# ESCOMP/POP2-CESM

Hardware: AMD Instinct MI355X
Metric: simulated_years_per_day (higher is better)
Workload: dtype f64; 1 GPU; tx0.1v3; nt=2, steps_per_day=300, step_calls_per_day=319, distribution=equal-block-counts, blocks_local=1, hmix=del4, hmix_tracer=del4, vmix=kpp, partial_bottom_cells=False, ns_boundary=closed, grid_input=False, tadvect=centered, solver=pcg, preconditioner=diagonal, transport=none, kpp_surface_buoyancy=on-demand down to the boundary-layer depth

## Files before the change

include/pop_amd.h:

```cpp
#ifndef POP_AMD_H
#define POP_AMD_H

#ifdef __cplusplus
extern "C" {
#endif

#define POP_CONFIG_VERSION 7
typedef struct pop_config {
  int struct_version;
  int nx_global, ny_global, km, nt;
  int block_size_x, block_size_y;
  int ew_boundary;
  int ns_boundary;
  int hmix_momentum;
  int hmix_tracer;
  int lvariable_hmix;
  int vmix_choice;
  int tadvect;
  int solver_choice;
  int max_iterations;
  int convergence_check_freq;
  int tmix_opt;
  int time_mix_freq;
  int steps_per_day;
// ... 104 lines not shown
  int evp_wave;
  int fpcg_a_pair;
  int kpp_sparse;
  int pbc_generic_thomas;
  int pbc_generic_kpp;
  int stream_priority;
  int gm_sf_stored;
  int state3d_levels;
  int pcg_persist;
  int gm_flux_tile;
  int pcsi_two_step;
  int block_sums_relay;
  int pcsi_evp_fused;
  int aniso_side;
  int submeso_all_levels;
} pop_tuning;
void pop_tuning_init(pop_tuning *t);
int pop_get_tuning(const pop_ctx *ctx, pop_tuning *resolved);

int pop_create(const pop_config *cfg, int rank, int nranks, int flags, pop_ctx **out);
typedef struct pop_grid_input {
  const double *ULAT, *ULON, *HTN, *HTE, *HUS, *HUW, *ANGLE;
  const int *KMT;
  const double *DZBC;
} pop_grid_input;
int pop_create_with_grid(const pop_config *cfg, const pop_grid_input *grid, int rank, int nranks, int flags, pop_ctx **out);
int pop_create_tuned(const pop_config *cfg, const pop_grid_input *grid, const pop_tuning *tuning, int rank, int nranks, int flags, pop_ctx **out);
int pop_read_grid_files(const char *horiz_grid_file, const char *topography_file, int nx_global, int ny_global,
                        double *seven_records , int *kmt );
int pop_destroy(pop_ctx *ctx);
// ... 82 lines not shown
```

pop2-cesm_amd/csrc/kernels_barotropic.hpp:

```cpp
#pragma once
#include "kernels_common.hpp"

namespace pop {

#define POP_RED_THREADS 256

struct BtropArgs {
  const double *ZX, *ZY, *GXC, *GXO, *GYC, *GYO, *UBO, *VBO, *PCUR, *FW, *PGUESS;
  double *UH, *VH, *W3, *W4, *RHS, *centerWgt, *PNEW, *GXN, *GYN, *UBN, *VBN;
  const double *GXR, *GYR;
  const double *scal;
  double rcheck, rconst;
};
__global__ void k_btrop_rhs1(DevGrid g, StepParams sp, BtropArgs a) {
  Col c;
  if (!col_setup(g, c, false)) return;
  const long long q = c.q2;
  double W3, W4;
  if (sp.leapfrogts) {
    W3 = sp.c2dtp * (a.ZX[q] - sp.gamma * a.GXC[q] - (1.0 - sp.gamma) * a.GXO[q]);
    W4 = sp.c2dtp * (a.ZY[q] - sp.gamma * a.GYC[q] - (1.0 - sp.gamma) * a.GYO[q]);
  } else {
    W3 = sp.c2dtp * (a.ZX[q] - a.GXC[q]);
    W4 = sp.c2dtp * (a.ZY[q] - a.GYC[q]);
// ... 600 lines not shown

}

namespace pop {

struct FusedArgs {
  double *X, *R, *Z, *S0, *S1, *Q;
  double *AZ; const double *A0R;
  const double *Bv, *C;
  double *partA, *partB;
  SolverScalars *sc;
  const int *srcmap;
  int nchunk, nblocks;
  const double *bsA, *bsB;
  int presummed;
  const int *sendmap, *send_off, *send_slot;
  double *sendbuf;
  const int *rmap;
  const double *rbuf;
};
__device__ __forceinline__ bool send_band(const DevGrid &g, int b, int i, int j) {
  return i + 1 < g.ib + NGHOST || i + 1 > blk_ie(g, b) - NGHOST || j + 1 < g.jb + NGHOST || j + 1 > blk_je(g, b) - NGHOST;
}
__device__ __forceinline__ void pack_cell(const FusedArgs &a, long long q, double val) {
  const int e = a.sendmap[q];
  if (e < 0) return;
  for (int n = a.send_off[e]; n < a.send_off[e + 1]; ++n) a.sendbuf[a.send_slot[n]] = val;
}
__device__ __forceinline__ double z_at(const FusedArgs &a, int m) {
  if (a.rmap) { const int rs = a.rmap[m]; if (rs >= 0) return a.rbuf[rs]; }
  return a.Z[m];
}

template <class T>
__device__ __forceinline__ T sld(const T *p) { return *(const __attribute__((address_space(4))) T *)p; }
__device__ __forceinline__ double presummed_total(const double *__restrict__ bs, int nblocks) {
  double total = 0.0;
  for (int b = 0; b < nblocks; ++b) total = total + sld(bs + b);
  return total;
}
__device__ __forceinline__ double fused_total(const double *__restrict__ partial, int nchunk, int nblocks,
                                              const double *__restrict__ bs, int presummed) {
  __shared__ double shf[POP_RED_THREADS];
  __shared__ double shf_tot;
  const int t = threadIdx.x;
  double total = 0.0;
  if (presummed) return presummed_total(bs, nblocks);
  for (int b = 0; b < nblocks; ++b) {
    double v = 0.0;
    for (int c = t; c < nchunk; c += POP_RED_THREADS) v = v + partial[(long long)b * nchunk + c];
    shf[t] = v;
    __syncthreads();
    if (t < 64) { const double x = tree_tail64((shf[t] + shf[t + 128]) + (shf[t + 64] + shf[t + 192])); if (t == 0) shf_tot = x; }
    __syncthreads();
    total = total + shf_tot;
  }
  return total;
}

constexpr unsigned long long POP_SPIN_EMPTY = 0x7FF8DEADBEEF0001ULL;

// ... 314 lines not shown
    a.X[q] = x + al * s;
    const double rn = r - al * qq;
    a.R[q] = rn;
    if (a.sendmap && send_band(g, b, i, j)) pack_cell(a, q, rn * a.A0R[q]);
  } else if (live && a.rmap) {
    const int rs = a.rmap[q];
    if (rs >= 0) {
      const double sg = a.rbuf[rs] + bt * a.S0[q];
      a.S0[q] = sg;
      a.X[q] = a.X[q] + al * sg;
    }
  }
}

template <bool XUPD>
__global__ void __launch_bounds__(POP_RED_THREADS / 2)
k_fpcg_b2(DevGrid g, FusedArgs a) {
  const int stop = sld(&a.sc->stop);
  const double alpha = XUPD ? sld(&a.sc->alpha) : 0.0;
  const double eta0 = sld(&a.sc->eta0);
  const double rz = presummed_total(a.bsA, a.nblocks);
  if (red_land_out<1>(g, a.partB, a.nchunk, a.sendmap != nullptr)) return;
  __shared__ double sh[POP_RED_THREADS];
  const int b = blockIdx.y, t = threadIdx.x, nxb = g.nxb;
  const long long p0 = (long long)red_chunk(g) * POP_RED_THREADS + 2 * t;
  const bool live0 = p0 < g.n2, live1 = p0 + 1 < g.n2;
  const int pp = live0 ? (int)p0 : 0;
  const int i = pp % nxb, j = pp / nxb;
  const long long q = (long long)b * g.n2 + pp;
  const bool fast = live1 && i + 1 > g.ib && i + 2 < blk_ie(g, b) && j + 1 > g.jb && j + 1 < blk_je(g, b);
  double v0 = 0.0, v1 = 0.0;
  double zr[3][4], sr[3][4];
  double2 cc, xx, x0, xm, y0, ym;
  double x0w = 0.0, xmw = 0.0, y0w = 0.0, ymw = 0.0, mk0 = 0.0, mk1 = 0.0;
  if (fast) {
#pragma unroll
    for (int r = 0; r < 3; ++r) {
      const long long o = q + (long long)(r - 1) * nxb;
      const double2 zc = *reinterpret_cast<const double2 *>(a.Z + o), sc = *reinterpret_cast<const double2 *>(a.S0 + o);
      zr[r][0] = a.Z[o - 1]; zr[r][1] = zc.x; zr[r][2] = zc.y; zr[r][3] = a.Z[o + 2];
      sr[r][0] = a.S0[o - 1]; sr[r][1] = sc.x; sr[r][2] = sc.y; sr[r][3] = a.S0[o + 2];
    }
    cc = *reinterpret_cast<const double2 *>(a.C + q);
    x0 = *reinterpret_cast<const double2 *>(g.XW + q); xm = *reinterpret_cast<const double2 *>(g.XW + q - nxb);
    y0 = *reinterpret_cast<const double2 *>(g.YW + q); ym = *reinterpret_cast<const double2 *>(g.YW + q - nxb);
    x0w = g.XW[q - 1]; xmw = g.XW[q - 1 - nxb]; y0w = g.YW[q - 1]; ymw = g.YW[q - 1 - nxb];
    mk0 = (double)g.mMask8[q]; mk1 = (double)g.mMask8[q + 1];
    if (XUPD) xx = *reinterpret_cast<const double2 *>(a.X + q);
  }
  if (stop) return;
  const double bt = rz / eta0;
  if (blockIdx.x == 0 && blockIdx.y == 0 && t == 0) { a.sc->eta1 = rz; a.sc->beta_cg = bt; }
  if (fast) {
    if (XUPD) *reinterpret_cast<double2 *>(a.X + q) = make_double2(xx.x + alpha * sr[1][1], xx.y + alpha * sr[1][2]);
    double2 no0, nom, ea0, ne0, nem;
    const double ne0w = x0w + y0w, nemw = xmw + ymw;
    ne0.x = x0.x + y0.x; ne0.y = x0.y + y0.y; nem.x = xm.x + ym.x; nem.y = xm.y + ym.y;
    const double eaw = x0w + xmw - y0w - ymw;
    ea0.x = x0.x + xm.x - y0.x - ym.x; ea0.y = x0.y + xm.y - y0.y - ym.y;
    no0.x = y0.x + y0w - x0.x - x0w; no0.y = y0.y + y0.x - x0.y - x0.x;
    nom.x = ym.x + ymw - xm.x - xmw; nom.y = ym.y + ym.x - xm.y - xm.x;
#define SN(r, c) (zr[r][c] + sr[r][c] * bt)
    const double sA = SN(1, 1), sB = SN(1, 2);
    double aqA = cc.x * sA;
    aqA = aqA + no0.x * SN(2, 1); aqA = aqA + nom.x * SN(0, 1); aqA = aqA + ea0.x * SN(1, 2); aqA = aqA + eaw * SN(1, 0);
    aqA = aqA + ne0.x * SN(2, 2); aqA = aqA + nem.x * SN(0, 2); aqA = aqA + ne0w * SN(2, 0); aqA = aqA + nemw * SN(0, 0);
    double aqB = cc.y * sB;
    aqB = aqB + no0.y * SN(2, 2); aqB = aqB + nom.y * SN(0, 2); aqB = aqB + ea0.y * SN(1, 3); aqB = aqB + ea0.x * SN(1, 1);
    aqB = aqB + ne0.y * SN(2, 3); aqB = aqB + nem.y * SN(0, 3); aqB = aqB + ne0.x * SN(2, 1); aqB = aqB + nem.x * SN(0, 1);
#undef SN
    *reinterpret_cast<double2 *>(a.S1 + q) = make_double2(sA, sB);
    *reinterpret_cast<double2 *>(a.Q + q) = make_double2(aqA, aqB);
    v0 = (aqA * sA) * mk0; v1 = (aqB * sB) * mk1;
  } else {
    const int off[9] = {0, nxb, -nxb, 1, -1, nxb + 1, -nxb + 1, nxb - 1, -nxb - 1};
    const long long qsafe = (long long)b * g.n2 + nxb + 1;
#pragma unroll
    for (int e = 0; e < 2; ++e) {
      const bool live = (e == 0 ? live0 : live1);
      const int p2 = live ? (int)(p0 + e) : 0, ii = p2 % nxb, jj = p2 / nxb;
      const long long qq = (long long)b * g.n2 + p2;
      const bool in_e = live && interior(g, b, ii, jj);
      const long long qn = in_e ? qq : qsafe;
      const double sold = a.S0[qq], xold = XUPD ? a.X[qq] : 0.0;
      const double zown = in_e ? a.Z[qq] : z_at(a, (int)qq);
      int m[9];
#pragma unroll
      for (int n = 1; n < 9; ++n) m[n] = a.srcmap[qn + off[n]];
      const double wv[9] = {a.C[qn], g.WNo[qn], g.WNo[qn - nxb], g.WEa[qn], g.WEa[qn - 1], g.WNE[qn], g.WNE[qn - nxb], g.WNE[qn - 1], g.WNE[qn - 1 - nxb]};
      const double mk = (double)g.mMask8[qn];
      double zn[9], sn0[9];
#pragma unroll
      for (int n = 1; n < 9; ++n) { const int mm = (m[n] >= 0) ? m[n] : (int)qn; zn[n] = z_at(a, mm); sn0[n] = a.S0[mm]; }
      const double s = zown + sold * bt;
      double aq = 0.0, vv = 0.0;
      if (in_e) {
        aq = wv[0] * s;
#pragma unroll
        for (int n = 1; n < 9; ++n) {
          const double sn = (m[n] >= 0) ? zn[n] + sn0[n] * bt : 0.0 + 0.0 * bt;
          aq = aq + wv[n] * sn;
        }
        vv = (aq * s) * mk;
      }
      if (live) {
        if (XUPD) a.X[qq] = xold + alpha * sold;
        a.S1[qq] = s; a.Q[qq] = aq;
      }
      if (e == 0) v0 = vv; else v1 = vv;
    }
  }
  sh[2 * t] = v0; sh[2 * t + 1] = v1;
  __syncthreads();
  if (t < 64) {
    const double x = tree_tail64((sh[t] + sh[t + 128]) + (sh[t + 64] + sh[t + 192]));
    if (t == 0) a.partB[(long long)b * a.nchunk + red_chunk(g)] = x;
  }
}

__global__ void __launch_bounds__(POP_RED_THREADS)
k_fpcg_xr(DevGrid g, FusedArgs a) {
  if (a.sc->stop) return;
  if (red_land(g, a.sendmap != nullptr)) return;
  const int p2 = red_cell(g), b = blockIdx.y;
  const double sq = fused_total(a.partB, a.nchunk, a.nblocks, a.bsB, a.presummed);
  const double rz = a.sc->eta1;
  const double alpha = rz / sq;
  if (blockIdx.x == 0 && blockIdx.y == 0 && threadIdx.x == 0) { a.sc->eta0 = rz; a.sc->alpha = alpha; }
  if (p2 >= g.n2) return;
  const long long q = (long long)b * g.n2 + p2;
  a.X[q] = a.X[q] + alpha * a.S0[q];
}

template <bool WITH_RR>
__global__ void __launch_bounds__(POP_RED_THREADS)
k_fresidual(DevGrid g, FusedArgs a) {
  if (a.sc->stop) return;
  if (WITH_RR ? red_land_out<1>(g, a.partA, a.nchunk, a.sendmap != nullptr) : red_land(g, a.sendmap != nullptr)) return;
  const int p2 = red_cell(g), b = blockIdx.y;
  double v[1] = {0.0};
// ... 116 lines not shown
```

pop2-cesm_amd/csrc/launch_solvers.hpp:

```cpp
#pragma once

namespace {

SolverArgs solver_args(pop_ctx *c) {
  SolverArgs a{};
  a.X = c->PS[c->newt]; a.R = c->R; a.S0 = c->S0; a.S1 = c->S1; a.Q = c->Q; a.Z = c->Z; a.AZ = c->AZ;
  a.Bv = c->RHS; a.C = c->centerWgt; a.partial = c->partial; a.sc = c->sc;
  return a;
}

int evp_apply(pop_ctx *c, const double *X, double *PX, bool residual = true) {
  const int wave = tun_or(c->h.tun.evp_wave, 3);
  if (wave == 3 && c->evp.C0 && residual)
    hipLaunchKernelGGL(k_evp_apply_wave3<true>, dim3((unsigned)((c->evp.S + POP_EVP_SB - 1) / POP_EVP_SB)), dim3(64), 0, c->stream, c->evp, c->g.nxb, X, PX);
  else if (wave == 3 && c->evp.C0)
    hipLaunchKernelGGL(k_evp_apply_wave3<false>, dim3((unsigned)((c->evp.S + POP_EVP_SB - 1) / POP_EVP_SB)), dim3(64), 0, c->stream, c->evp, c->g.nxb, X, PX);
  else if (wave == 2 && c->evp.C0)
    hipLaunchKernelGGL(k_evp_apply_wave2, dim3((unsigned)((c->evp.S + POP_EVP_SB - 1) / POP_EVP_SB)), dim3(64), 0, c->stream, c->evp, c->g.nxb, X, PX);
  else if (wave != 0)
    hipLaunchKernelGGL(k_evp_apply_wave, dim3((unsigned)((c->evp.S + POP_EVP_SB - 1) / POP_EVP_SB)), dim3(64), 0, c->stream, c->evp, c->g.nxb, X, PX);
  else
    hipLaunchKernelGGL(k_evp_apply, dim3((unsigned)((c->evp.S + POP_EVP_THREADS - 1) / POP_EVP_THREADS)), dim3(POP_EVP_THREADS), 0, c->stream,
                       c->evp, c->g.nxb, X, PX);
  HIPCHK(c, hipGetLastError());
// ... 51 lines not shown
      if (read_scalars(c, &s)) return 1;
      rr = s.rr;
      if (rr < c->h.convergenceCriterion) { c->numIterations = m; break; }
    }
  }
  if (pending) { a = solver_args(c); hipLaunchKernelGGL(k_pcg_xr, G, B, 0, c->stream, c->g, a); }
  return solver_finish(c, nullptr, nullptr, 0, rr, "POP_SolversPCG");
}

static bool fpcg_pair_ok(const pop_ctx *c, const SolveView &v, const FusedArgs &a) {
  return v.g.red_act && a.presummed && !a.sendmap && (v.g.red_nact % 16) == 0 && !tun_off(c->h.tun.fpcg_b2) && !tun_off(c->h.tun.fpcg_a_pair);
}
static bool presum_by_size(long long nchunk, long long nblocks) { return nchunk * nblocks > 2048; }
static bool two_cell_shape(const DevGrid &g, bool presummed) { return presummed && (g.nxb & 1) == 0 && !g.red_tiles; }
static bool two_cell_ok(const pop_ctx *c, const DevGrid &g, bool presummed) { return two_cell_shape(g, presummed) && !tun_off(c->h.tun.fpcg_b2); }
FusedArgs fused_args(pop_ctx *c, const SolveView &v) {
  FusedArgs a{};
  a.X = v.X; a.R = v.R; a.Z = v.Z; a.S0 = v.S0; a.S1 = v.S1; a.Q = v.Q;
  a.Bv = v.RHS; a.C = v.C; a.partA = v.partial; a.partB = v.partial + (size_t)v.nchunk * v.g.nblocks;
  a.sc = c->sc; a.srcmap = v.srcmap; a.nchunk = v.nchunk; a.nblocks = v.g.nblocks;
  a.bsA = v.blocksum + 2 * v.nblocks_tot; a.bsB = v.blocksum + 3 * v.nblocks_tot;
  a.presummed = (presum_by_size(v.nchunk, v.g.nblocks) || tun_on(c->h.tun.solver_presum)) ? 1 : 0;
  return a;
}
constexpr int POP_RELAY_LMAX = 36;
static bool presum_relay(const pop_ctx *c, const SolveView &v) {
  const int terms = (v.nchunk + POP_RED_THREADS - 1) / POP_RED_THREADS;
  const int t = tun_or(c->h.tun.block_sums_relay, 1);
  return (terms > 64 || t == 2) && (terms + 3) / 4 <= POP_RELAY_LMAX && t != 0;
}
template <int NF = 1>
void presum(pop_ctx *c, const SolveView &v, const double *partial, double *bs) {
  if (presum_relay(c, v)) hipLaunchKernelGGL((k_block_sums_relay<NF, POP_RELAY_LMAX>), dim3(v.g.nblocks, NF), dim3(1024), 0, c->stream, partial, v.nchunk, (const int *)c->iota, bs);
  else hipLaunchKernelGGL(k_block_sums<NF>, dim3(v.g.nblocks), dim3(POP_RED_THREADS), 0, c->stream, partial, v.nchunk, (const int *)c->iota, bs);
}
dim3 view_grid(const SolveView &v) { return dim3(red_grid_x(v.g), v.g.nblocks); }
template <bool WITH_RR>
// ... 13 lines not shown
    else hipLaunchKernelGGL(k_fpcg_a_pair<false>, GP, B, 0, c->stream, v.g, a);
  } else if (update) hipLaunchKernelGGL(k_fpcg_a<true>, G, B, 0, c->stream, v.g, a);
  else hipLaunchKernelGGL(k_fpcg_a<false>, G, B, 0, c->stream, v.g, a);
}
void launch_fpcg_b(pop_ctx *c, const SolveView &v, const FusedArgs &a, bool xupd) {
  const dim3 G = view_grid(v);
  const bool two = two_cell_ok(c, v.g, a.presummed != 0);
  if (two && xupd) hipLaunchKernelGGL(k_fpcg_b2<true>, G, dim3(POP_RED_THREADS / 2), 0, c->stream, v.g, a);
  else if (two) hipLaunchKernelGGL(k_fpcg_b2<false>, G, dim3(POP_RED_THREADS / 2), 0, c->stream, v.g, a);
  else if (xupd) hipLaunchKernelGGL(k_fpcg_b<true>, G, dim3(POP_RED_THREADS), 0, c->stream, v.g, a);
  else hipLaunchKernelGGL(k_fpcg_b<false>, G, dim3(POP_RED_THREADS), 0, c->stream, v.g, a);
}
void fused_iterations(pop_ctx *c, SolveView &v, int n, bool pending) {
  for (int it = 0; it < n; ++it) {
    FusedArgs a = fused_args(c, v);
    launch_fpcg_a(c, v, a, pending);
    if (a.presummed) presum(c, v, a.partA, (double *)a.bsA);
    launch_fpcg_b(c, v, a, pending);
    if (a.presummed) presum(c, v, a.partB, (double *)a.bsB);
    std::swap(v.S0, v.S1);
    pending = true;
  }
}
int fused_interval(pop_ctx *c, SolveView &v, int freq) {
  const dim3 G = view_grid(v), B(POP_RED_THREADS);
  fused_iterations(c, v, freq, false);
  FusedArgs a = fused_args(c, v);
  hipLaunchKernelGGL(k_fpcg_xr, G, B, 0, c->stream, v.g, a);
  launch_fresidual<true>(c, v, a);
  hipLaunchKernelGGL(k_rr_total, dim3(1), dim3(POP_RED_THREADS), 0, c->stream, (const double *)v.partial, v.nchunk, v.g.nblocks, c->sc, c->host_rr, c->h.convergenceCriterion);
// ... 173 lines not shown
}
int persist_give_up(pop_ctx *c, const char *instead, const SolveView &v, const double *X0) {
  c->persist_gave_up += 1;
  fprintf(stderr, "libpop_amd: %s -- continuing with %s\n", c->err.c_str(), instead);
  c->err.clear();
  if (X0) HIPCHK(c, hipMemcpyAsync(v.X, X0, sizeof(double) * v.g.n2 * v.g.nblocks, hipMemcpyDeviceToDevice, c->stream));
  return 0;
}
int persist_keep_x0(pop_ctx *c, const SolveView &v, const pop_ctx::PersistPlan &pl) {
  HIPCHK(c, hipMemcpyAsync(pl.X0, v.X, sizeof(double) * v.g.n2 * v.g.nblocks, hipMemcpyDeviceToDevice, c->stream));
  return 0;
}

int solver_pcg_fused(pop_ctx *c, SolveView &v) {
  const pop_config &cf = c->h.c;
  c->persist_used = 0;
  if (!tun_off(c->h.tun.pcg_persist) && !fused_args(c, v).presummed) {
    const pop_ctx::PersistPlan *pl = c->persist_gave_up ? nullptr : persist_plan(c, v);
    if (pl) {
      static void (*const kern[4])(PersistArgs) = {k_pcg_persist<1>, k_pcg_persist<2>, k_pcg_persist<4>, k_pcg_persist<8>};
      if (persist_keep_x0(c, v, *pl)) return 1;
      const int e = persist_launch(c, v, *pl, persist_args(c, v, *pl), kern, "resident pcg", "POP_SolversPCG");
      if (e != 3) return e;
      if (persist_give_up(c, "the two-launch pcg", v, pl->X0)) return 1;
    }
  }
  const dim3 G = view_grid(v), B(POP_RED_THREADS);
  const int freq = cf.convergence_check_freq;
  if (solver_begin(c, 1.0)) return 1;
  HIPCHK(c, hipMemsetAsync(v.S0, 0, sizeof(double) * v.g.n2 * v.g.nblocks, c->stream));
  launch_fresidual<false>(c, v, fused_args(c, v));
  c->numIterations = cf.max_iterations;
// ... 587 lines not shown
```

pop2-cesm_amd/csrc/pop_amd.hip:

```cpp
#include <hip/hip_runtime.h>
#include <algorithm>
#include <chrono>
#include <unordered_map>
#include "kernels_baroclinic.hpp"
#include "kernels_barotropic.hpp"
#include "kernels_mix.hpp"
#include "kernels_thomas_reg.hpp"
#include "kernels_momentum_lds.hpp"
#include "kernels_aniso.hpp"
#include "kernels_submeso.hpp"
#include "kernels_tracer_lds.hpp"
#include "kernels_rf.hpp"
#include "kernels_pcsi.hpp"
#include "kernels_evp.hpp"
#include "kernels_lwlim.hpp"
#include "kernels_gm.hpp"
#include "kernels_pcg_persist.hpp"
#include <fcntl.h>
#include <unistd.h>
#include "rccl_transport.hpp"

using namespace pop;

#include "pop_ctx.hpp"
// ... 79 lines not shown
  return pop_create_tuned(cfg, grid, nullptr, rank, nranks, flags, out);
}

#define POP_TUNING_FIELDS(X)                                                                                                            \
  X(land_skip, "POP_LAND_SKIP") X(land_full_steps, "POP_LAND_FULL_STEPS") X(xcd_remap, "POP_XCD_REMAP") X(red_tiles, "POP_RED_TILES")   \
  X(red_band, "POP_RED_BAND") X(lds_order, "POP_LDS_ORDER") X(momentum_lds, "POP_MOMENTUM_LDS") X(tracer_lds, "POP_TRACER_LDS")         \
  X(generic_thomas, "POP_GENERIC_THOMAS") X(reg_thomas_t, "POP_REG_THOMAS_T") X(thomas_pair, "POP_THOMAS_PAIR")                         \
  X(tracer_fwd, "POP_TRACER_FWD") X(vdc_shared, "POP_VDC_SHARED") X(side_stream, "POP_SIDE_STREAM") X(del4_side, "POP_DEL4_SIDE")       \
  X(del4_tile, "POP_DEL4_TILE") X(d2t_fuse, "POP_D2T_FUSE") X(d2u_fuse, "POP_D2U_FUSE") X(vmixu_defer, "POP_VMIXU_DEFER")               \
  X(vmixu_inline, "POP_VMIXU_INLINE") X(btrop_inline, "POP_BTROP_INLINE") X(kpp_ahead, "POP_KPP_AHEAD") X(kpp_col, "POP_KPP_COL")       \
  X(kpp_lazy, "POP_KPP_LAZY") X(kpp_ushear_hint, "POP_KPP_USHEAR_HINT") X(kpp_ushear_margin, "POP_KPP_USHEAR_MARGIN")                   \
  X(kpp_side_stream, "POP_KPP_SIDE_STREAM") X(kpp_buoy_waves, "POP_KPP_BUOY_WAVES") X(kpp_interior_generic, "POP_KPP_INTERIOR_GENERIC") \
  X(kpp_src_full, "POP_KPP_SRC_FULL") X(solver_unfused, "POP_SOLVER_UNFUSED") X(solver_nograph, "POP_SOLVER_NOGRAPH")                   \
  X(solver_presum, "POP_SOLVER_PRESUM") X(solver_distributed, "POP_SOLVER_DISTRIBUTED") X(solver_overlap_off, "POP_SOLVER_OVERLAP_OFF") \
  X(fpcg_b2, "POP_FPCG_B2") X(pcsi_step2, "POP_PCSI_STEP2") X(halo_separate, "POP_HALO_SEPARATE")                                       \
  X(halo_overlap_off, "POP_HALO_OVERLAP_OFF") X(rccl_overlap, "POP_RCCL_OVERLAP") X(evp_wave, "POP_EVP_WAVE") X(fpcg_a_pair, "POP_FPCG_A_PAIR") X(stream_priority, "POP_STREAM_PRIORITY") X(kpp_sparse, "POP_KPP_SPARSE") X(pbc_generic_thomas, "POP_PBC_GENERIC_THOMAS") X(pbc_generic_kpp, "POP_PBC_GENERIC_KPP") X(state3d_levels, "POP_STATE3D_LEVELS") X(gm_sf_stored, "POP_GM_SF_STORED") X(pcg_persist, "POP_PCG_PERSIST") X(gm_flux_tile, "POP_GM_FLUX_TILE") X(pcsi_two_step, "POP_PCSI_TWO_STEP") X(block_sums_relay, "POP_BLOCK_SUMS_RELAY") X(pcsi_evp_fused, "POP_PCSI_EVP_FUSED") X(aniso_side, "POP_ANISO_SIDE") X(submeso_all_levels, "POP_SUBMESO_ALL_LEVELS")
void pop_tuning_init(pop_tuning *t) {
  if (!t) return;
  t->struct_bytes = (int)sizeof(pop_tuning);
#define X(f, e) t->f = POP_TUNING_UNSET;
  POP_TUNING_FIELDS(X)
#undef X
}
static void tuning_resolve(pop_tuning &t, const pop_tuning *user) {
  pop_tuning_init(&t);
  if (user && user->struct_bytes == (int)sizeof(pop_tuning)) t = *user;
  auto env = [](const char *name, int &v) {
    const char *e = getenv(name);
    if (!e) return;
    char *end = nullptr;
    const long x = strtol(e, &end, 10);
// ... 439 lines not shown
      for (size_t w = act[b].size(); w < longest; ++w) seq.push_back(land[b][w - act[b].size()]);
      const size_t per = longest / 8;
      for (size_t w = 0; w < longest; ++w) list[(size_t)b * longest + (w % per) * 8 + w / per] = seq[w];
    }
    if (!can_pad) longest = (size_t)nc;
    if (longest < (size_t)nc) {
      std::vector<int> cnt(h.nblocks);
      for (int b = 0; b < h.nblocks; ++b) cnt[b] = (int)act[b].size();
      if (dev_upload(c, &c->red_act, list.data(), list.size()) || dev_upload(c, &c->red_cnt, cnt.data(), cnt.size())) return 1;
      c->red_nact = (int)longest;
    }
  }
  if (dev_alloc(c, &c->partial, (size_t)c->nchunk * h.nblocks * 2 + POP_RELAY_SLACK) || dev_alloc(c, &c->blocksum, (size_t)h.nblocks_tot * 4)) return 1;
  { std::vector<int> io(h.nblocks_tot); for (int b = 0; b < h.nblocks_tot; ++b) io[b] = b; if (dev_upload(c, &c->iota, io.data(), io.size())) return 1; }
  if (dev_alloc(c, &c->sc, 1)) return 1;
  { std::vector<int> gid(h.nblocks); for (int lb = 0; lb < h.nblocks; ++lb) gid[lb] = h.local_ids[lb] - 1; if (dev_upload(c, &c->gid, gid.data(), gid.size())) return 1; }
  { std::vector<int> log(h.nblocks_tot, -1); for (int lb = 0; lb < h.nblocks; ++lb) log[h.local_ids[lb] - 1] = lb; if (dev_upload(c, &c->loc_of_gid, log.data(), log.size())) return 1; }
  c->ncopy = (int)h.halo.copy_dst.size(); c->nfill = (int)h.halo.fill_dst.size();
  if (c->ncopy && (dev_upload(c, &c->copy_dst, h.halo.copy_dst.data(), c->ncopy) || dev_upload(c, &c->copy_src, h.halo.copy_src.data(), c->ncopy))) return 1;
  if (c->nfill && dev_upload(c, &c->fill_dst, h.halo.fill_dst.data(), c->nfill)) return 1;
  for (auto &pp : h.halo.peers) {
    DevPeer d; d.rank = pp.rank; d.nsend = (int)pp.send_src.size(); d.nrecv = (int)pp.recv_dst.size();
    if (d.nsend && dev_upload(c, &d.send_src, pp.send_src.data(), d.nsend)) return 1;
    if (d.nrecv && dev_upload(c, &d.recv_dst, pp.recv_dst.data(), d.nrecv)) return 1;
    c->peers.push_back(d);
  }
  if (cfg->ns_boundary == 2) {
    size_t nmax = 1;
    for (int loc = 0; loc < 5; ++loc) {
      const TripolePlan &T = h.halo.tripole[loc];
// ... 248 lines not shown
  if (n == "d2t_fused") return c->d2t_next[0] != nullptr;
  if (n == "d2u_fused") return c->d2u_next[0] != nullptr;
  if (n == "d2t_last_formed") return c->d2t_last_formed;
  if (n == "d2u_last_formed") return c->d2u_last_formed;
  if (n == "avg_ts") return c->avg_ts;
  if (n == "nsteps_total") return c->nsteps_total;
  if (n == "nsteps_per_interval") return c->h.nsteps_per_interval;
  if (n == "solver_stream_ops") return (int)c->solver_ops;
  if (n == "solver_iterations_enqueued") return (int)c->solver_enq;
  if (n == "rank") return c->h.rank;
  if (n == "nranks") return c->h.nranks;
  if (n == "solver_chunks_per_block") return c->nchunk;
  if (n == "solver_chunks_listed") return c->red_act ? c->red_nact : -1;
  if (n == "solver_chunks_active") return c->red_active_total;
  if (n == "pcg_persist_used") return c->persist_used;
  if (n == "pcg_persist_gave_up") return c->persist_gave_up;
  if (n == "pcsi_evp_fused") return c->pcsi_evp_fused ? 1 : 0;
  if (n == "pcsi_two_step") return (c->pcsi_two_step || c->pcsi_two_step_dist) ? 1 : 0;
  if (n == "pcg_persist_workgroups") return c->persist_nwg;
  if (n == "pcg_persist_chunks_per_workgroup") return c->persist_cp;
  if (n == "solver_path") return c->host_only ? 0 : solver_path_code(c);
  if (n == "thomas_register_tracers") return c->reg_thomas_t && (c->g.km == 60 || c->g.km == 62);
  if (n == "thomas_register_velocity") return c->reg_thomas && (c->g.km == 60 || c->g.km == 62);
  if (n == "max_blocks_per_rank") return c->max_blocks_per_rank;
  if (n == "ocean_columns_local") return (int)c->h.ocean_cols_local;
  if (n == "ocean_columns_total") return (int)c->h.ocean_cols_total;
  return -1;
}
double pop_get_scalar(const pop_ctx *c, const char *name) {
  const std::string n(name);
// ... 1340 lines not shown
```

pop2-cesm_amd/csrc/pop_ctx.hpp:

```cpp
#pragma once

#define HIPCHK(ctx, call)                                                                       \
  do {                                                                                          \
    hipError_t e_ = (call);                                                                     \
    if (e_ != hipSuccess) {                                                                     \
      (ctx)->err = std::string(#call) + ": " + hipGetErrorString(e_);                           \
      return 1;                                                                                 \
    }                                                                                           \
  } while (0)

struct PhaseTimer { double ms = 0; int calls = 0; };

struct DevPeer { int rank; int *send_src = nullptr, *recv_dst = nullptr; int nsend = 0, nrecv = 0; };

struct pop_ctx {
  HostModel h;
  bool host_only = true;
  std::string err;
  hipStream_t stream = nullptr;
  bool own_stream = false;
  DevGrid g{};
  std::map<std::string, double *> d2;
  std::map<std::string, int *> di2;
  std::vector<void *> allocs;
// ... 41 lines not shown
  struct PersistPlan {
    const void *key = nullptr; bool ok = false; std::string why;
    int CP = 0, nwg = 0, nwin_max = 0, nslots = 0;
    int *own_q = nullptr, *halo_off = nullptr, *halo_q = nullptr; unsigned short *nbr = nullptr;
    PWord *W = nullptr;
    double *X0 = nullptr;
  };
  unsigned long long persist_epoch = 0;
  std::vector<PersistPlan> persist;
  std::vector<int> h_srcmap;
  double *persist_out = nullptr;
  int persist_used = 0;
  int persist_gave_up = 0;
  int red_active_total = 0;
  int persist_nwg = 0, persist_cp = 0;
  bool pcsi_two_cell = false;
  bool pcsi_two_step = false;
  bool pcsi_two_step_dist = false;
  double *pcsi_raw = nullptr;
  int *pcsi_jfold = nullptr;
  bool pcsi_evp_fused = false;
  bool reg_thomas_t = true;
  int trc_lds_rows = 4;
  int mom_lds_rows = 4;
  bool reg_thomas = true;
  SolveView gv{};
  double *gTAREA = nullptr; int *gKMT = nullptr;
  int nchunk = 0, numIterations = 0;
  double rmsResidual = 0.0;
  int *copy_dst = nullptr, *copy_src = nullptr, *fill_dst = nullptr;
// ... 111 lines not shown
```

Baseline: 10.22 SYPD.

## Add accumulator-owner fused PCG kernels that replace per-iteration presum reduction launches

```diff
diff --git a/include/pop_amd.h b/include/pop_amd.h
--- a/include/pop_amd.h
+++ b/include/pop_amd.h
@@ -142,6 +142,7 @@
   int pcsi_evp_fused;
   int aniso_side;
   int submeso_all_levels;
+  int fpcg_acc_owner;
 } pop_tuning;
 void pop_tuning_init(pop_tuning *t);
 int pop_get_tuning(const pop_ctx *ctx, pop_tuning *resolved);
diff --git a/pop2-cesm_amd/csrc/kernels_barotropic.hpp b/pop2-cesm_amd/csrc/kernels_barotropic.hpp
--- a/pop2-cesm_amd/csrc/kernels_barotropic.hpp
+++ b/pop2-cesm_amd/csrc/kernels_barotropic.hpp
@@ -638,6 +638,7 @@
   int nchunk, nblocks;
   const double *bsA, *bsB;
   int presummed;
+  double *accA, *accB;
   const int *sendmap, *send_off, *send_slot;
   double *sendbuf;
   const int *rmap;
@@ -663,12 +664,27 @@
   for (int b = 0; b < nblocks; ++b) total = total + sld(bs + b);
   return total;
 }
+__device__ __forceinline__ double acc_total(const double *__restrict__ acc, int nblocks) {
+  const int l = threadIdx.x & 63;
+  double total = 0.0;
+  for (int b = 0; b < nblocks; ++b) {
+    const double *__restrict__ v = acc + (long long)b * POP_RED_THREADS;
+    const double x = tree_tail64((v[l] + v[l + 128]) + (v[l + 64] + v[l + 192]));
+    total = total + __shfl(x, 0, 64);
+  }
+  return total;
+}
 __device__ __forceinline__ double fused_total(const double *__restrict__ partial, int nchunk, int nblocks,
-                                              const double *__restrict__ bs, int presummed) {
+                                              const double *__restrict__ bs, int presummed, const double *__restrict__ acc = nullptr) {
   __shared__ double shf[POP_RED_THREADS];
   __shared__ double shf_tot;
   const int t = threadIdx.x;
   double total = 0.0;
+  if (acc) {
+    if (t < 64) { const double x = acc_total(acc, nblocks); if (t == 0) shf_tot = x; }
+    __syncthreads();
+    return shf_tot;
+  }
   if (presummed) return presummed_total(bs, nblocks);
   for (int b = 0; b < nblocks; ++b) {
     double v = 0.0;
@@ -1013,6 +1029,120 @@
 }
 
 template <bool XUPD>
+struct FpcgBPair {
+  long long p0, q;
+  int nxb;
+  bool live0, live1, fast;
+  double zr[3][4], sr[3][4];
+  double2 cc, xx, x0, xm, y0, ym;
+  double x0w, xmw, y0w, ymw, mk0, mk1;
+  __device__ __forceinline__ void setup(const DevGrid &g, int b, int chunk, int tt) {
+    nxb = g.nxb;
+    p0 = (long long)chunk * POP_RED_THREADS + 2 * tt;
+    live0 = p0 < g.n2; live1 = p0 + 1 < g.n2;
+    const int pp = live0 ? (int)p0 : 0;
+    const int i = pp % nxb, j = pp / nxb;
+    q = (long long)b * g.n2 + pp;
+    fast = live1 && i + 1 > g.ib && i + 2 < blk_ie(g, b) && j + 1 > g.jb && j + 1 < blk_je(g, b);
+    x0w = 0.0; xmw = 0.0; y0w = 0.0; ymw = 0.0; mk0 = 0.0; mk1 = 0.0;
+  }
+  __device__ __forceinline__ void load(const DevGrid &g, const FusedArgs &a, int b, int chunk, int tt) {
+    setup(g, b, chunk, tt);
+    if (fast) load_fast(g, a);
+  }
+  __device__ __forceinline__ void finish(const DevGrid &g, const FusedArgs &a, int b, double bt, double alpha, double &v0, double &v1) {
+    if (fast) finish_fast(a, bt, alpha, v0, v1);
+    else finish_generic(g, a, b, bt, alpha, v0, v1);
+  }
+  __device__ __forceinline__ void run(const DevGrid &g, const FusedArgs &a, int b, int chunk, int tt, double bt, double alpha, double &v0, double &v1) {
+    setup(g, b, chunk, tt);
+    if (fast) { load_fast(g, a); finish_fast(a, bt, alpha, v0, v1); }
+    else finish_generic(g, a, b, bt, alpha, v0, v1);
+  }
+  __device__ __forceinline__ void load_fast(const DevGrid &g, const FusedArgs &a) {
+    {
+#pragma unroll
+      for (int r = 0; r < 3; ++r) {
+        const long long o = q + (long long)(r - 1) * nxb;
+        const double2 zc = *reinterpret_cast<const double2 *>(a.Z + o), sc = *reinterpret_cast<const double2 *>(a.S0 + o);
+        zr[r][0] = a.Z[o - 1]; zr[r][1] = zc.x; zr[r][2] = zc.y; zr[r][3] = a.Z[o + 2];
+        sr[r][0] = a.S0[o - 1]; sr[r][1] = sc.x; sr[r][2] = sc.y; sr[r][3] = a.S0[o + 2];
+      }
+      cc = *reinterpret_cast<const double2 *>(a.C + q);
+      x0 = *reinterpret_cast<const double2 *>(g.XW + q); xm = *reinterpret_cast<const double2 *>(g.XW + q - nxb);
+      y0 = *reinterpret_cast<const double2 *>(g.YW + q); ym = *reinterpret_cast<const double2 *>(g.YW + q - nxb);
+      x0w = g.XW[q - 1]; xmw = g.XW[q - 1 - nxb]; y0w = g.YW[q - 1]; ymw = g.YW[q - 1 - nxb];
+      mk0 = (double)g.mMask8[q]; mk1 = (double)g.mMask8[q + 1];
+      if (XUPD) xx = *reinterpret_cast<const double2 *>(a.X + q);
+    }
+  }
+  __device__ __forceinline__ void finish_fast(const FusedArgs &a, double bt, double alpha, double &v0, double &v1) {
+    {
+      if (XUPD) *reinterpret_cast<double2 *>(a.X + q) = make_double2(xx.x + alpha * sr[1][1], xx.y + alpha * sr[1][2]);
+      double2 no0, nom, ea0, ne0, nem;
+      const double ne0w = x0w + y0w, nemw = xmw + ymw;
+      ne0.x = x0.x + y0.x; ne0.y = x0.y + y0.y; nem.x = xm.x + ym.x; nem.y = xm.y + ym.y;
+      const double eaw = x0w + xmw - y0w - ymw;
+      ea0.x = x0.x + xm.x - y0.x - ym.x; ea0.y = x0.y + xm.y - y0.y - ym.y;
+      no0.x = y0.x + y0w - x0.x - x0w; no0.y = y0.y + y0.x - x0.y - x0.x;
+      nom.x = ym.x + ymw - xm.x - xmw; nom.y = ym.y + ym.x - xm.y - xm.x;
+#define SN(r, c) (zr[r][c] + sr[r][c] * bt)
+      const double sA = SN(1, 1), sB = SN(1, 2);
+      double aqA = cc.x * sA;
+      aqA = aqA + no0.x * SN(2, 1); aqA = aqA + nom.x * SN(0, 1); aqA = aqA + ea0.x * SN(1, 2); aqA = aqA + eaw * SN(1, 0);
+      aqA = aqA + ne0.x * SN(2, 2); aqA = aqA + nem.x * SN(0, 2); aqA = aqA + ne0w * SN(2, 0); aqA = aqA + nemw * SN(0, 0);
+      double aqB = cc.y * sB;
+      aqB = aqB + no0.y * SN(2, 2); aqB = aqB + nom.y * SN(0, 2); aqB = aqB + ea0.y * SN(1, 3); aqB = aqB + ea0.x * SN(1, 1);
+      aqB = aqB + ne0.y * SN(2, 3); aqB = aqB + nem.y * SN(0, 3); aqB = aqB + ne0.x * SN(2, 1); aqB = aqB + nem.x * SN(0, 1);
+#undef SN
+      *reinterpret_cast<double2 *>(a.S1 + q) = make_double2(sA, sB);
+      *reinterpret_cast<double2 *>(a.Q + q) = make_double2(aqA, aqB);
+      v0 = (aqA * sA) * mk0; v1 = (aqB * sB) * mk1;
+    }
+  }
+  __device__ __forceinline__ void finish_generic(const DevGrid &g, const FusedArgs &a, int b, double bt, double alpha, double &v0, double &v1) {
+    v0 = 0.0; v1 = 0.0;
+    {
+      const int off[9] = {0, nxb, -nxb, 1, -1, nxb + 1, -nxb + 1, nxb - 1, -nxb - 1};
+      const long long qsafe = (long long)b * g.n2 + nxb + 1;
+#pragma unroll
+      for (int e = 0; e < 2; ++e) {
+        const bool live = (e == 0 ? live0 : live1);
+        const int p2 = live ? (int)(p0 + e) : 0, ii = p2 % nxb, jj = p2 / nxb;
+        const long long qq = (long long)b * g.n2 + p2;
+        const bool in_e = live && interior(g, b, ii, jj);
+        const long long qn = in_e ? qq : qsafe;
+        const double sold = a.S0[qq], xold = XUPD ? a.X[qq] : 0.0;
+        const double zown = in_e ? a.Z[qq] : z_at(a, (int)qq);
+        int m[9];
+#pragma unroll
+        for (int n = 1; n < 9; ++n) m[n] = a.srcmap[qn + off[n]];
+        const double wv[9] = {a.C[qn], g.WNo[qn], g.WNo[qn - nxb], g.WEa[qn], g.WEa[qn - 1], g.WNE[qn], g.WNE[qn - nxb], g.WNE[qn - 1], g.WNE[qn - 1 - nxb]};
+        const double mk = (double)g.mMask8[qn];
+        double zn[9], sn0[9];
+#pragma unroll
+        for (int n = 1; n < 9; ++n) { const int mm = (m[n] >= 0) ? m[n] : (int)qn; zn[n] = z_at(a, mm); sn0[n] = a.S0[mm]; }
+        const double s = zown + sold * bt;
+        double aq = 0.0, vv = 0.0;
+        if (in_e) {
+          aq = wv[0] * s;
+#pragma unroll
+          for (int n = 1; n < 9; ++n) {
+            const double sn = (m[n] >= 0) ? zn[n] + sn0[n] * bt : 0.0 + 0.0 * bt;
+            aq = aq + wv[n] * sn;
+          }
+          vv = (aq * s) * mk;
+        }
+        if (live) {
+          if (XUPD) a.X[qq] = xold + alpha * sold;
+          a.S1[qq] = s; a.Q[qq] = aq;
+        }
+        if (e == 0) v0 = vv; else v1 = vv;
+      }
+    }
+  }
+};
+template <bool XUPD>
 __global__ void __launch_bounds__(POP_RED_THREADS / 2)
 k_fpcg_b2(DevGrid g, FusedArgs a) {
   const int stop = sld(&a.sc->stop);
@@ -1021,94 +1151,14 @@
   const double rz = presummed_total(a.bsA, a.nblocks);
   if (red_land_out<1>(g, a.partB, a.nchunk, a.sendmap != nullptr)) return;
   __shared__ double sh[POP_RED_THREADS];
-  const int b = blockIdx.y, t = threadIdx.x, nxb = g.nxb;
-  const long long p0 = (long long)red_chunk(g) * POP_RED_THREADS + 2 * t;
-  const bool live0 = p0 < g.n2, live1 = p0 + 1 < g.n2;
-  const int pp = live0 ? (int)p0 : 0;
-  const int i = pp % nxb, j = pp / nxb;
-  const long long q = (long long)b * g.n2 + pp;
-  const bool fast = live1 && i + 1 > g.ib && i + 2 < blk_ie(g, b) && j + 1 > g.jb && j + 1 < blk_je(g, b);
-  double v0 = 0.0, v1 = 0.0;
-  double zr[3][4], sr[3][4];
-  double2 cc, xx, x0, xm, y0, ym;
-  double x0w = 0.0, xmw = 0.0, y0w = 0.0, ymw = 0.0, mk0 = 0.0, mk1 = 0.0;
-  if (fast) {
-#pragma unroll
-    for (int r = 0; r < 3; ++r) {
-      const long long o = q + (long long)(r - 1) * nxb;
-      const double2 zc = *reinterpret_cast<const double2 *>(a.Z + o), sc = *reinterpret_cast<const double2 *>(a.S0 + o);
-      zr[r][0] = a.Z[o - 1]; zr[r][1] = zc.x; zr[r][2] = zc.y; zr[r][3] = a.Z[o + 2];
-      sr[r][0] = a.S0[o - 1]; sr[r][1] = sc.x; sr[r][2] = sc.y; sr[r][3] = a.S0[o + 2];
-    }
-    cc = *reinterpret_cast<const double2 *>(a.C + q);
-    x0 = *reinterpret_cast<const double2 *>(g.XW + q); xm = *reinterpret_cast<const double2 *>(g.XW + q - nxb);
-    y0 = *reinterpret_cast<const double2 *>(g.YW + q); ym = *reinterpret_cast<const double2 *>(g.YW + q - nxb);
-    x0w = g.XW[q - 1]; xmw = g.XW[q - 1 - nxb]; y0w = g.YW[q - 1]; ymw = g.YW[q - 1 - nxb];
-    mk0 = (double)g.mMask8[q]; mk1 = (double)g.mMask8[q + 1];
-    if (XUPD) xx = *reinterpret_cast<const double2 *>(a.X + q);
-  }
+  const int b = blockIdx.y, t = threadIdx.x;
+  FpcgBPair<XUPD> P;
+  P.load(g, a, b, red_chunk(g), t);
   if (stop) return;
   const double bt = rz / eta0;
   if (blockIdx.x == 0 && blockIdx.y == 0 && t == 0) { a.sc->eta1 = rz; a.sc->beta_cg = bt; }
-  if (fast) {
-    if (XUPD) *reinterpret_cast<double2 *>(a.X + q) = make_double2(xx.x + alpha * sr[1][1], xx.y + alpha * sr[1][2]);
-    double2 no0, nom, ea0, ne0, nem;
-    const double ne0w = x0w + y0w, nemw = xmw + ymw;
-    ne0.x = x0.x + y0.x; ne0.y = x0.y + y0.y; nem.x = xm.x + ym.x; nem.y = xm.y + ym.y;
-    const double eaw = x0w + xmw - y0w - ymw;
-    ea0.x = x0.x + xm.x - y0.x - ym.x; ea0.y = x0.y + xm.y - y0.y - ym.y;
-    no0.x = y0.x + y0w - x0.x - x0w; no0.y = y0.y + y0.x - x0.y - x0.x;
-    nom.x = ym.x + ymw - xm.x - xmw; nom.y = ym.y + ym.x - xm.y - xm.x;
-#define SN(r, c) (zr[r][c] + sr[r][c] * bt)
-    const double sA = SN(1, 1), sB = SN(1, 2);
-    double aqA = cc.x * sA;
-    aqA = aqA + no0.x * SN(2, 1); aqA = aqA + nom.x * SN(0, 1); aqA = aqA + ea0.x * SN(1, 2); aqA = aqA + eaw * SN(1, 0);
-    aqA = aqA + ne0.x * SN(2, 2); aqA = aqA + nem.x * SN(0, 2); aqA = aqA + ne0w * SN(2, 0); aqA = aqA + nemw * SN(0, 0);
-    double aqB = cc.y * sB;
-    aqB = aqB + no0.y * SN(2, 2); aqB = aqB + nom.y * SN(0, 2); aqB = aqB + ea0.y * SN(1, 3); aqB = aqB + ea0.x * SN(1, 1);
-    aqB = aqB + ne0.y * SN(2, 3); aqB = aqB + nem.y * SN(0, 3); aqB = aqB + ne0.x * SN(2, 1); aqB = aqB + nem.x * SN(0, 1);
-#undef SN
-    *reinterpret_cast<double2 *>(a.S1 + q) = make_double2(sA, sB);
-    *reinterpret_cast<double2 *>(a.Q + q) = make_double2(aqA, aqB);
-    v0 = (aqA * sA) * mk0; v1 = (aqB * sB) * mk1;
-  } else {
-    const int off[9] = {0, nxb, -nxb, 1, -1, nxb + 1, -nxb + 1, nxb - 1, -nxb - 1};
-    const long long qsafe = (long long)b * g.n2 + nxb + 1;
-#pragma unroll
-    for (int e = 0; e < 2; ++e) {
-      const bool live = (e == 0 ? live0 : live1);
-      const int p2 = live ? (int)(p0 + e) : 0, ii = p2 % nxb, jj = p2 / nxb;
-      const long long qq = (long long)b * g.n2 + p2;
-      const bool in_e = live && interior(g, b, ii, jj);
-      const long long qn = in_e ? qq : qsafe;
-      const double sold = a.S0[qq], xold = XUPD ? a.X[qq] : 0.0;
-      const double zown = in_e ? a.Z[qq] : z_at(a, (int)qq);
-      int m[9];
-#pragma unroll
-      for (int n = 1; n < 9; ++n) m[n] = a.srcmap[qn + off[n]];
-      const double wv[9] = {a.C[qn], g.WNo[qn], g.WNo[qn - nxb], g.WEa[qn], g.WEa[qn - 1], g.WNE[qn], g.WNE[qn - nxb], g.WNE[qn - 1], g.WNE[qn - 1 - nxb]};
-      const double mk = (double)g.mMask8[qn];
-      double zn[9], sn0[9];
-#pragma unroll
-      for (int n = 1; n < 9; ++n) { const int mm = (m[n] >= 0) ? m[n] : (int)qn; zn[n] = z_at(a, mm); sn0[n] = a.S0[mm]; }
-      const double s = zown + sold * bt;
-      double aq = 0.0, vv = 0.0;
-      if (in_e) {
-        aq = wv[0] * s;
-#pragma unroll
-        for (int n = 1; n < 9; ++n) {
-          const double sn = (m[n] >= 0) ? zn[n] + sn0[n] * bt : 0.0 + 0.0 * bt;
-          aq = aq + wv[n] * sn;
-        }
-        vv = (aq * s) * mk;
-      }
-      if (live) {
-        if (XUPD) a.X[qq] = xold + alpha * sold;
-        a.S1[qq] = s; a.Q[qq] = aq;
-      }
-      if (e == 0) v0 = vv; else v1 = vv;
-    }
-  }
+  double v0, v1;
+  P.finish(g, a, b, bt, alpha, v0, v1);
   sh[2 * t] = v0; sh[2 * t + 1] = v1;
   __syncthreads();
   if (t < 64) {
@@ -1117,12 +1167,134 @@
   }
 }
 
+constexpr int POP_ACC_THREADS = 1024;
+constexpr int POP_ACC_MAXTERMS = 1024;
+__device__ __forceinline__ int acc_of_workgroup(int w) { return (w & 7) * (POP_RED_THREADS / 8) + (w >> 3); }
+__device__ __forceinline__ bool own_land(const DevGrid &g, int b, int k) {
+  return g.skip && !(b == 0 && k == 0) && land_run(g, b, (long long)k * POP_RED_THREADS, POP_RED_THREADS);
+}
+__device__ __forceinline__ double wave_uniform(double x) {
+  const long long u = __double_as_longlong(x);
+  const unsigned lo = __builtin_amdgcn_readfirstlane((unsigned)u), hi = __builtin_amdgcn_readfirstlane((unsigned)(u >> 32));
+  return __longlong_as_double((long long)(((unsigned long long)hi << 32) | lo));
+}
+template <class F>
+__device__ __forceinline__ void own_chunks(const DevGrid &g, int b, int acc, int nchunk, double *part, F chunk_partial) {
+  const int l = threadIdx.x & 63, wave = __builtin_amdgcn_readfirstlane((int)(threadIdx.x >> 6)), nwaves = (int)(blockDim.x >> 6);
+  int turn = 0;
+  for (int m0 = 0; acc + POP_RED_THREADS * m0 < nchunk; m0 += 64) {
+    const int chl = acc + POP_RED_THREADS * (m0 + l);
+    const bool there = chl < nchunk, land = there && own_land(g, b, chl);
+    if (wave == 0 && land) part[m0 + l] = 0.0;
+    unsigned long long todo = __ballot(there && !land);
+    while (todo) {
+      const int bit = __ffsll(todo) - 1;
+      todo &= todo - 1;
+      const bool mine = turn % nwaves == wave;
+      ++turn;
+      if (mine) {
+        const double x = chunk_partial(acc + POP_RED_THREADS * (m0 + bit));
+        if (l == 0) part[m0 + bit] = x;
+      }
+    }
+  }
+}
+__device__ __forceinline__ void own_store_acc(const double *part, int acc, int nchunk, double *__restrict__ out) {
+  if (threadIdx.x != 0) return;
+  const int terms = (nchunk - acc + POP_RED_THREADS - 1) / POP_RED_THREADS;
+  double v = 0.0;
+  int m = 0;
+  for (; m + 16 <= terms; m += 16) {
+    double w[16];
+#pragma unroll
+    for (int u = 0; u < 16; ++u) w[u] = part[m + u];
+#pragma unroll
+    for (int u = 0; u < 16; ++u) v = v + w[u];
+  }
+  for (; m < terms; ++m) v = v + part[m];
+  *out = v;
+}
+template <bool UPDATE>
+__global__ void __launch_bounds__(POP_ACC_THREADS)
+k_fpcg_a_own(DevGrid g, FusedArgs a) {
+  __shared__ double part[POP_ACC_MAXTERMS];
+  if (sld(&a.sc->stop)) return;
+  const int b = blockIdx.y, l = threadIdx.x & 63, acc = acc_of_workgroup(blockIdx.x);
+  double alpha = 0.0;
+  if (UPDATE) {
+    const double sq = acc_total(a.accB, a.nblocks);
+    const double rz = sld(&a.sc->eta1);
+    alpha = wave_uniform(rz / sq);
+    if (blockIdx.x == 0 && blockIdx.y == 0 && threadIdx.x == 0) { a.sc->eta0 = rz; a.sc->alpha = alpha; }
+  }
+  own_chunks(g, b, acc, a.nchunk, part, [&](int ch) {
+    long long q[4]; bool live[4];
+    double r[4], qq[4] = {0.0, 0.0, 0.0, 0.0}, cw[4], mk[4], v[4];
+#pragma unroll
+    for (int u = 0; u < 4; ++u) {
+      const long long p2 = (long long)ch * POP_RED_THREADS + l + 64 * u;
+      live[u] = p2 < g.n2;
+      q[u] = (long long)b * g.n2 + (live[u] ? p2 : 0);
+    }
+#pragma unroll
+    for (int u = 0; u < 4; ++u) {
+      r[u] = a.R[q[u]];
+      if (UPDATE) qq[u] = a.Q[q[u]];
+      cw[u] = a.C[q[u]]; mk[u] = (double)g.mMask8[q[u]];
+    }
+#pragma unroll
+    for (int u = 0; u < 4; ++u) {
+      v[u] = 0.0;
+      if (live[u]) {
+        const int p2 = (int)(q[u] - (long long)b * g.n2);
+        const int i = p2 % g.nxb, j = p2 / g.nxb;
+        double rr = r[u];
+        if (UPDATE) { rr = rr - alpha * qq[u]; a.R[q[u]] = rr; }
+        const double z = (cw[u] != 0.0) ? rr / cw[u] : 0.0;
+        a.Z[q[u]] = z;
+        if (interior(g, b, i, j)) v[u] = (rr * z) * mk[u];
+      }
+    }
+    return tree_tail64((v[0] + v[2]) + (v[1] + v[3]));
+  });
+  __syncthreads();
+  own_store_acc(part, acc, a.nchunk, a.accA + (long long)b * POP_RED_THREADS + acc);
+}
+template <bool XUPD>
+__global__ void __launch_bounds__(POP_ACC_THREADS)
+k_fpcg_b_own(DevGrid g, FusedArgs a) {
+  __shared__ double part[POP_ACC_MAXTERMS];
+  if (sld(&a.sc->stop)) return;
+  const double alpha = XUPD ? sld(&a.sc->alpha) : 0.0;
+  const double eta0 = sld(&a.sc->eta0);
+  const int b = blockIdx.y, l = threadIdx.x & 63, acc = acc_of_workgroup(blockIdx.x);
+  const double rz = acc_total(a.accA, a.nblocks);
+  const double bt = wave_uniform(rz / eta0);
+  if (blockIdx.x == 0 && blockIdx.y == 0 && threadIdx.x == 0) { a.sc->eta1 = rz; a.sc->beta_cg = bt; }
+  const bool odd = (l & 1) != 0;
+  own_chunks(g, b, acc, a.nchunk, part, [&](int ch) {
+    double s02 = 0.0, s13 = 0.0;
+#pragma unroll 1
+    for (int h = 0; h < 2; ++h) {
+      FpcgBPair<XUPD> P;
+      double v0, v1;
+      P.run(g, a, b, ch, (l >> 1) + 64 * (l & 1) + 32 * h, bt, alpha, v0, v1);
+      const double mine = odd ? v1 : v0, theirs = __shfl_xor(odd ? v0 : v1, 1, 64);
+      const double lo = odd ? theirs : mine, hi = odd ? mine : theirs;
+      if (h == 0) s02 = lo + hi; else s13 = lo + hi;
+    }
+    return tree_tail64(s02 + s13);
+  });
+  __syncthreads();
+  own_store_acc(part, acc, a.nchunk, a.accB + (long long)b * POP_RED_THREADS + acc);
+}
+
 __global__ void __launch_bounds__(POP_RED_THREADS)
 k_fpcg_xr(DevGrid g, FusedArgs a) {
   if (a.sc->stop) return;
   if (red_land(g, a.sendmap != nullptr)) return;
   const int p2 = red_cell(g), b = blockIdx.y;
-  const double sq = fused_total(a.partB, a.nchunk, a.nblocks, a.bsB, a.presummed);
+  const double sq = fused_total(a.partB, a.nchunk, a.nblocks, a.bsB, a.presummed, a.accB);
   const double rz = a.sc->eta1;
   const double alpha = rz / sq;
   if (blockIdx.x == 0 && blockIdx.y == 0 && threadIdx.x == 0) { a.sc->eta0 = rz; a.sc->alpha = alpha; }
diff --git a/pop2-cesm_amd/csrc/launch_solvers.hpp b/pop2-cesm_amd/csrc/launch_solvers.hpp
--- a/pop2-cesm_amd/csrc/launch_solvers.hpp
+++ b/pop2-cesm_amd/csrc/launch_solvers.hpp
@@ -89,6 +89,13 @@
 static bool presum_by_size(long long nchunk, long long nblocks) { return nchunk * nblocks > 2048; }
 static bool two_cell_shape(const DevGrid &g, bool presummed) { return presummed && (g.nxb & 1) == 0 && !g.red_tiles; }
 static bool two_cell_ok(const pop_ctx *c, const DevGrid &g, bool presummed) { return two_cell_shape(g, presummed) && !tun_off(c->h.tun.fpcg_b2); }
+static bool fpcg_acc_owner_ok(const pop_ctx *c, const SolveView &v) {
+  const int t = c->h.tun.fpcg_acc_owner;
+  const int terms = (v.nchunk + POP_RED_THREADS - 1) / POP_RED_THREADS;
+  if (tun_off(t) || tun_off(c->h.tun.fpcg_b2) || !c->fpcg_acc || c->h.nranks != 1 || v.srcmap != c->srcmap) return false;
+  if (!two_cell_shape(v.g, true) || terms > POP_ACC_MAXTERMS) return false;
+  return t == 2 || presum_by_size(v.nchunk, v.g.nblocks);
+}
 FusedArgs fused_args(pop_ctx *c, const SolveView &v) {
   FusedArgs a{};
   a.X = v.X; a.R = v.R; a.Z = v.Z; a.S0 = v.S0; a.S1 = v.S1; a.Q = v.Q;
@@ -96,6 +103,7 @@
   a.sc = c->sc; a.srcmap = v.srcmap; a.nchunk = v.nchunk; a.nblocks = v.g.nblocks;
   a.bsA = v.blocksum + 2 * v.nblocks_tot; a.bsB = v.blocksum + 3 * v.nblocks_tot;
   a.presummed = (presum_by_size(v.nchunk, v.g.nblocks) || tun_on(c->h.tun.solver_presum)) ? 1 : 0;
+  if (fpcg_acc_owner_ok(c, v)) { a.accA = c->fpcg_acc; a.accB = c->fpcg_acc + (size_t)POP_RED_THREADS * v.g.nblocks; }
   return a;
 }
 constexpr int POP_RELAY_LMAX = 36;
@@ -139,6 +147,15 @@
 void fused_iterations(pop_ctx *c, SolveView &v, int n, bool pending) {
   for (int it = 0; it < n; ++it) {
     FusedArgs a = fused_args(c, v);
+    if (a.accA) {
+      const dim3 G(POP_RED_THREADS, v.g.nblocks), B(POP_ACC_THREADS);
+      if (pending) { hipLaunchKernelGGL(k_fpcg_a_own<true>, G, B, 0, c->stream, v.g, a); hipLaunchKernelGGL(k_fpcg_b_own<true>, G, B, 0, c->stream, v.g, a); }
+      else { hipLaunchKernelGGL(k_fpcg_a_own<false>, G, B, 0, c->stream, v.g, a); hipLaunchKernelGGL(k_fpcg_b_own<false>, G, B, 0, c->stream, v.g, a); }
+      c->acc_owner_used = 1;
+      std::swap(v.S0, v.S1);
+      pending = true;
+      continue;
+    }
     launch_fpcg_a(c, v, a, pending);
     if (a.presummed) presum(c, v, a.partA, (double *)a.bsA);
     launch_fpcg_b(c, v, a, pending);
@@ -342,8 +359,8 @@
 
 int solver_pcg_fused(pop_ctx *c, SolveView &v) {
   const pop_config &cf = c->h.c;
-  c->persist_used = 0;
-  if (!tun_off(c->h.tun.pcg_persist) && !fused_args(c, v).presummed) {
+  c->persist_used = 0; c->acc_owner_used = 0;
+  if (!tun_off(c->h.tun.pcg_persist) && !fused_args(c, v).presummed && !fused_args(c, v).accA) {
     const pop_ctx::PersistPlan *pl = c->persist_gave_up ? nullptr : persist_plan(c, v);
     if (pl) {
       static void (*const kern[4])(PersistArgs) = {k_pcg_persist<1>, k_pcg_persist<2>, k_pcg_persist<4>, k_pcg_persist<8>};
diff --git a/pop2-cesm_amd/csrc/pop_amd.hip b/pop2-cesm_amd/csrc/pop_amd.hip
--- a/pop2-cesm_amd/csrc/pop_amd.hip
+++ b/pop2-cesm_amd/csrc/pop_amd.hip
@@ -117,7 +117,7 @@
   X(kpp_src_full, "POP_KPP_SRC_FULL") X(solver_unfused, "POP_SOLVER_UNFUSED") X(solver_nograph, "POP_SOLVER_NOGRAPH")                   \
   X(solver_presum, "POP_SOLVER_PRESUM") X(solver_distributed, "POP_SOLVER_DISTRIBUTED") X(solver_overlap_off, "POP_SOLVER_OVERLAP_OFF") \
   X(fpcg_b2, "POP_FPCG_B2") X(pcsi_step2, "POP_PCSI_STEP2") X(halo_separate, "POP_HALO_SEPARATE")                                       \
-  X(halo_overlap_off, "POP_HALO_OVERLAP_OFF") X(rccl_overlap, "POP_RCCL_OVERLAP") X(evp_wave, "POP_EVP_WAVE") X(fpcg_a_pair, "POP_FPCG_A_PAIR") X(stream_priority, "POP_STREAM_PRIORITY") X(kpp_sparse, "POP_KPP_SPARSE") X(pbc_generic_thomas, "POP_PBC_GENERIC_THOMAS") X(pbc_generic_kpp, "POP_PBC_GENERIC_KPP") X(state3d_levels, "POP_STATE3D_LEVELS") X(gm_sf_stored, "POP_GM_SF_STORED") X(pcg_persist, "POP_PCG_PERSIST") X(gm_flux_tile, "POP_GM_FLUX_TILE") X(pcsi_two_step, "POP_PCSI_TWO_STEP") X(block_sums_relay, "POP_BLOCK_SUMS_RELAY") X(pcsi_evp_fused, "POP_PCSI_EVP_FUSED") X(aniso_side, "POP_ANISO_SIDE") X(submeso_all_levels, "POP_SUBMESO_ALL_LEVELS")
+  X(halo_overlap_off, "POP_HALO_OVERLAP_OFF") X(rccl_overlap, "POP_RCCL_OVERLAP") X(evp_wave, "POP_EVP_WAVE") X(fpcg_a_pair, "POP_FPCG_A_PAIR") X(stream_priority, "POP_STREAM_PRIORITY") X(kpp_sparse, "POP_KPP_SPARSE") X(pbc_generic_thomas, "POP_PBC_GENERIC_THOMAS") X(pbc_generic_kpp, "POP_PBC_GENERIC_KPP") X(state3d_levels, "POP_STATE3D_LEVELS") X(gm_sf_stored, "POP_GM_SF_STORED") X(pcg_persist, "POP_PCG_PERSIST") X(gm_flux_tile, "POP_GM_FLUX_TILE") X(pcsi_two_step, "POP_PCSI_TWO_STEP") X(block_sums_relay, "POP_BLOCK_SUMS_RELAY") X(pcsi_evp_fused, "POP_PCSI_EVP_FUSED") X(aniso_side, "POP_ANISO_SIDE") X(submeso_all_levels, "POP_SUBMESO_ALL_LEVELS") X(fpcg_acc_owner, "POP_FPCG_ACC_OWNER")
 void pop_tuning_init(pop_tuning *t) {
   if (!t) return;
   t->struct_bytes = (int)sizeof(pop_tuning);
@@ -587,6 +587,7 @@
   if (dev_alloc(c, &c->partial, (size_t)c->nchunk * h.nblocks * 2 + POP_RELAY_SLACK) || dev_alloc(c, &c->blocksum, (size_t)h.nblocks_tot * 4)) return 1;
   { std::vector<int> io(h.nblocks_tot); for (int b = 0; b < h.nblocks_tot; ++b) io[b] = b; if (dev_upload(c, &c->iota, io.data(), io.size())) return 1; }
   if (dev_alloc(c, &c->sc, 1)) return 1;
+  if (dev_alloc(c, &c->fpcg_acc, (size_t)2 * POP_RED_THREADS * h.nblocks)) return 1;
   { std::vector<int> gid(h.nblocks); for (int lb = 0; lb < h.nblocks; ++lb) gid[lb] = h.local_ids[lb] - 1; if (dev_upload(c, &c->gid, gid.data(), gid.size())) return 1; }
   { std::vector<int> log(h.nblocks_tot, -1); for (int lb = 0; lb < h.nblocks; ++lb) log[h.local_ids[lb] - 1] = lb; if (dev_upload(c, &c->loc_of_gid, log.data(), log.size())) return 1; }
   c->ncopy = (int)h.halo.copy_dst.size(); c->nfill = (int)h.halo.fill_dst.size();
@@ -865,6 +866,7 @@
   if (n == "solver_chunks_listed") return c->red_act ? c->red_nact : -1;
   if (n == "solver_chunks_active") return c->red_active_total;
   if (n == "pcg_persist_used") return c->persist_used;
+  if (n == "fpcg_acc_owner_used") return c->acc_owner_used;
   if (n == "pcg_persist_gave_up") return c->persist_gave_up;
   if (n == "pcsi_evp_fused") return c->pcsi_evp_fused ? 1 : 0;
   if (n == "pcsi_two_step") return (c->pcsi_two_step || c->pcsi_two_step_dist) ? 1 : 0;
diff --git a/pop2-cesm_amd/csrc/pop_ctx.hpp b/pop2-cesm_amd/csrc/pop_ctx.hpp
--- a/pop2-cesm_amd/csrc/pop_ctx.hpp
+++ b/pop2-cesm_amd/csrc/pop_ctx.hpp
@@ -79,6 +79,8 @@
   int persist_gave_up = 0;
   int red_active_total = 0;
   int persist_nwg = 0, persist_cp = 0;
+  double *fpcg_acc = nullptr;
+  int acc_owner_used = 0;
   bool pcsi_two_cell = false;
   bool pcsi_two_step = false;
   bool pcsi_two_step_dist = false;
```

After: 9.526 SYPD. 6.8% lower.
